# leggedrobotics/wild_visual_navigation

Hardware: AMD Instinct MI355X
Metric: frames/sec (448x448 DINO-ViT-S/8 + seg + MLP train-step) (higher is better)
Workload: dtype fp16 + e5m2-MX-correction linears (a w = a_h w_h + 2^-12 (a_h8 w_l8 + a_l8 w_h8); ~16 significand bits per product) + f16 attention products (two-plane q in the first six blocks), fp32 accumulate / residual (<= 1e-3 parity mode)

## Files before the change

wild_visual_navigation_amd/csrc/gemm_a384_x3.hip:

```cpp
#include <stdlib.h>

#include <algorithm>
#include <type_traits>

#include "common.h"
#include "wvn_internal.h"

namespace {

constexpr int KD = 384;
constexpr int BNT = 64;
constexpr int SLK = 128;
constexpr int NSL = KD / SLK;
constexpr int NS = 3;
constexpr int PLANE_BYTES = BNT * SLK * 2;
constexpr int SLICE_BYTES = 2 * PLANE_BYTES;
constexpr int RING_BYTES = NS * SLICE_BYTES;
constexpr int IMG_BF16 = 32 * 144;
constexpr int STG_BYTES = 2 * 64 * 80;
constexpr int STG_OFF = RING_BYTES;
constexpr int BIAS_OFF = STG_OFF + 4 * STG_BYTES;
constexpr int BM = 128;
constexpr int PIECES = SLICE_BYTES / 1024 / 4;
static_assert(PIECES == 8, "one DMA piece per k-step of a slice");
// ... 327 lines not shown
      if constexpr (TR) {
        const int c = 32 * t + 8 * g + 4 * hi + h2;
        if constexpr (EPI == X_GELU || EPI == X_GELU_FRAG) gelu_pair(v0, v1);
        if constexpr (EPI == X_GELU_FRAG && MX) {
          typedef __attribute__((ext_vector_type(2))) _Float16 h2_t;
          const uint32_t h = pack_f16x2(v0, v1);
          const h2_t hh = __builtin_bit_cast(h2_t, h);
          fragh[2 * (g & 1) + (h2 >> 1)] = h;
          {
            typedef __attribute__((ext_vector_type(2))) float f2_t;
            const f2_t res = f2_t{v0, v1} - f2_t{(float)hh[0], (float)hh[1]};
            frag8l[s >> 1] = mx_pk8(frag8l[s >> 1], res[0], res[1], MX_RES_INV, s & 1);
          }
          if ((s & 3) == 3) {
            const unsigned so = __builtin_amdgcn_readfirstlane((((m0w >> 5) * (p.N >> 4)) + 4 * jp + 2 * t + (g >> 1)) * 1024);
            wvn_store_b128_guarded(fragh, rs_c, lane * 16, so);
          }
          if (s == 7) {
            const unsigned so8 = __builtin_amdgcn_readfirstlane((((m0w >> 5) * (p.N >> 6)) + jp) * 2048 + t * 1024);
            wvn_store_b128_guarded(frag8l, rs_c2, lane * 16, so8);
          }
          return;
        }
        if constexpr (EPI == X_GELU_FRAG) {
          uint32_t h, l;
          split2(v0, v1, h, l);
          const int e = 2 * (g & 1) + (h2 >> 1);
          fragh[e] = h; fragl[e] = l;
          if ((s & 3) == 3) {
            const unsigned so = __builtin_amdgcn_readfirstlane((((m0w >> 5) * (p.N >> 4)) + 4 * jp + 2 * t + (g >> 1)) * 1024);
            wvn_store_b128_guarded(fragh, rs_c, lane * 16, so);
            wvn_store_b128_guarded(fragl, rs_c2, lane * 16, so);
          }
          return;
        }
        if constexpr (HEAD) {
          const wvn_f32x2_t b2 = *(const wvn_f32x2_t*)(bias_l + n0 + c);
          v0 += b2[0]; v1 += b2[1];
        }
        if constexpr (HEAD && !CODE) { v0 = fmaxf(v0, 0.f); v1 = fmaxf(v1, 0.f); }
        if constexpr (CODE) {
          const wvn_f32x2_t o = {v0, v1};
          *(wvn_f32x2_t*)(stg + l31 * 272 + c * 4) = o;
        } else if constexpr (EPI == X_RESID) {
          if (p.ls) { v0 *= p.ls[n0 + c]; v1 *= p.ls[n0 + c + 1]; }
          const wvn_f32x2_t o = {v0, v1};
          *(wvn_f32x2_t*)(stg + l31 * 272 + c * 4) = o;
        } else if constexpr (IS_QKV && F16OUT) {
          const float qs = n0 < p.heads * 64 ? p.q_scale : 1.f;
          uint32_t h, l;
          wvn_split2_f16(v0 * qs, v1 * qs, h, l);
          *(uint32_t*)(stg + l31 * 144 + c * 2) = h;
          *(uint32_t*)(stg + IMG_BF16 + l31 * 144 + c * 2) = l;
        } else {
          uint32_t h, l;
          split2(v0, v1, h, l);
          *(uint32_t*)(stg + l31 * 144 + c * 2) = h;
          *(uint32_t*)(stg + IMG_BF16 + l31 * 144 + c * 2) = l;
        }
      } else {
        const int mloc = 16 * (g >> 1) + 8 * hi + 4 * (g & 1) + h2;
        if constexpr (F16OUT) {
          *(uint32_t*)(stg + (32 * t + l31) * 80 + mloc * 2) = pack_f16x2(v0, v1);
        } else {
          uint32_t h, l;
          split2(v0, v1, h, l);
          *(uint32_t*)(stg + (32 * t + l31) * 80 + mloc * 2) = h;
          *(uint32_t*)(stg + 64 * 80 + (32 * t + l31) * 80 + mloc * 2) = l;
        }
      }
      return;
    }
    if constexpr (CODE) {
      const int it = s;
      const unsigned so = __builtin_amdgcn_readfirstlane(((m0w + 4 * it) * p.ld_code + (n0 - KD)) * 4);
      const u32x4_t o = *(const u32x4_t*)(stg + stg_rd_code + it * 4 * 272);
      const unsigned vo = m0w + 4 * it + (lane >> 4) < p.M ? voff[1] : OOB;
      wvn_store_b128_guarded(o, rs_code, vo, so);
    } else if constexpr (EPI == X_RESID) {
      const int it = s;
      const unsigned so = __builtin_amdgcn_readfirstlane(((m0w + 4 * it) * p.ldc + n0) * 4);
      f32x4_t v = *(const f32x4_t*)(stg + stg_rd + it * 4 * 272);
      const u32x4_t r = resid_q[it & 1];
      if (it + 2 < 8)
        resid_q[it & 1] = __builtin_amdgcn_raw_buffer_load_b128(rs_c, voff[0], __builtin_amdgcn_readfirstlane(((m0w + 4 * (it + 2)) * p.ldc + n0) * 4), 0);
#pragma unroll
      for (int e = 0; e < 4; ++e) v[e] += __uint_as_float(r[e]);
      u32x4_t o;
#pragma unroll
      for (int e = 0; e < 4; ++e) o[e] = __float_as_uint(v[e]);
      wvn_store_b128_guarded(o, rs_c, voff[0], so);
    } else if constexpr (IS_QKV && TR) {
      const int it = s & 3, pl = s >> 2;
      const int D = p.heads * 64;
      const int which = n0 / D, head = (n0 - which * D) >> 6;
      const unsigned so = __builtin_amdgcn_readfirstlane((which == 0 ? p.q_off : p.k_off) + head * p.npad * 64 * 2);
      const u32x4_t val = *(const u32x4_t*)(stg + pl * IMG_BF16 + ((lane >> 3) + it * 8) * 144 + (lane & 7) * 16);
      if (pl == 0) wvn_store_b128_guarded(val, rs_c, voff[it >> 1], so + (it & 1) * 1024);
      else {
        const bool keep = !F16OUT || (which == 0 && p.q_lo_f16);
        wvn_store_b128_guarded(val, rs_c2, keep ? voff[it >> 1] : OOB, so + (it & 1) * 1024);
      }
    } else if constexpr (IS_QKV && !TR) {
      const int it = s & 3, pl = s >> 2;
      if (pl == 1 && F16OUT) return;
      const int head = (MERGED ? n0 - 2 * p.heads * 64 : n0) >> 6;
      const u32x4_t val = *(const u32x4_t*)(stg + pl * 64 * 80 + ((lane >> 2) + it * 16) * 80 + (lane & 3) * 16);
      const unsigned so = __builtin_amdgcn_readfirstlane(p.v_off + (head * 64 + it * 16) * p.npad * 2);
      if (pl == 0) wvn_store_b128_guarded(val, rs_c, vt_off, so);
      else wvn_store_b128_guarded(val, rs_c2, vt_off, so);
    } else if constexpr (EPI == X_GELU_FRAG) {
    } else {
      const int it = s >> 1, pl = s & 1;
      const unsigned so = __builtin_amdgcn_readfirstlane(((m0w + 8 * it) * p.ldc + n0) * 2);
      const u32x4_t val = *(const u32x4_t*)(stg + pl * IMG_BF16 + stg_rd + it * 8 * 144);
      const unsigned vo = m0w + 8 * it + (lane >> 3) < p.M ? voff[0] : OOB;
      if (pl == 0) wvn_store_b128_guarded(val, rs_c, vo, so);
      else wvn_store_b128_guarded(val, rs_c2, vo, so);
    }
  };

  auto init_acc = [&](int j, auto tr_tag) __attribute__((always_inline)) {
    constexpr bool TR = decltype(tr_tag)::value;
    const int n0 = j * BNT;
    if constexpr (HEAD) {
#pragma unroll
      for (int t = 0; t < 2; ++t)
#pragma unroll
        for (int r = 0; r < 16; ++r) acc[t][r] = 0.f;
    } else if constexpr (TR) {
#pragma unroll
      for (int t = 0; t < 2; ++t)
#pragma unroll
        for (int g = 0; g < 4; ++g) {
          const f32x4_t b4 = *(const f32x4_t*)(bias_l + n0 + 32 * t + 8 * g + 4 * hi);
#pragma unroll
          for (int e = 0; e < 4; ++e) acc[t][4 * g + e] = b4[e];
        }
    } else {
#pragma unroll
      for (int t = 0; t < 2; ++t) {
        const float b = bias_l[n0 + 32 * t + l31];
#pragma unroll
        for (int r = 0; r < 16; ++r) acc[t][r] = b;
      }
    }
  };

  constexpr int ST2 = EPI == X_RESID ? 14 : (EPI == X_GELU || EPI == X_PLANES ? 8 : (EPI == X_GELU_FRAG ? 0 : (F16OUT ? 4 : 8)));
  constexpr int ST01 = EPI == X_GELU_FRAG ? (MX ? 3 : 4) : 0;
  long long t_wait = 0, t_iss = 0, t_mfma = 0;
  const long long t_start = TIMING ? (long long)__builtin_amdgcn_s_memtime() : 0;
  auto period = [&](int i, int ks, int j, bool stores_in_window, auto mtr, auto etr, auto epi_tag) __attribute__((always_inline)) {
    constexpr bool do_epi = decltype(epi_tag)::value;
    long long c0 = 0, c1 = 0, c2 = 0;
    if constexpr (TIMING) c0 = (long long)__builtin_amdgcn_s_memtime();
    if (i + 1 < total) {
      if (ks == 0 && stores_in_window && ST2 > 0) asm volatile("s_waitcnt vmcnt(%0)" ::"n"(PIECES + ST2) : "memory");
      else if (ks != 0 && do_epi && ST01 > 0) asm volatile("s_waitcnt vmcnt(%0)" ::"n"(PIECES + ST01) : "memory");
      else asm volatile("s_waitcnt vmcnt(%0)" ::"n"(PIECES) : "memory");
    } else {
      asm volatile("s_waitcnt vmcnt(0)" ::: "memory");
    }
    __builtin_amdgcn_s_barrier();
    if constexpr (TIMING) c1 = (long long)__builtin_amdgcn_s_memtime();
    issue_begin();
    __builtin_amdgcn_sched_barrier(0);
    if constexpr (TIMING) c2 = (long long)__builtin_amdgcn_s_memtime();
    if constexpr (BURST) {
#pragma unroll
      for (int s = 0; s < 8; ++s) issue_piece(i + NS - 1, s);
      __builtin_amdgcn_sched_barrier(0);
    }
    frag_read(i % NS, 0, 0);
#pragma unroll
    for (int s = 0; s < 8; ++s) {
      if constexpr (MX) {
        if (s + 1 < 8) frag_read(i % NS, s + 1, (s & 1) ^ 1);
        __builtin_amdgcn_sched_barrier(0);
      }
      if constexpr (!BURST) issue_piece(i + NS - 1, s);
      mfma_step(i % NS, ks, s, mtr);
      if constexpr (do_epi) epi_chunk(ks, j - 1, s, etr);
      if constexpr (MX) {
#pragma unroll
        for (int n = 0; n < 2; ++n) {
          __builtin_amdgcn_sched_group_barrier(0x008, 1, 0);
          __builtin_amdgcn_sched_group_barrier(0x002, 8, 0);
          __builtin_amdgcn_sched_group_barrier(0x200, 2, 0);
          __builtin_amdgcn_sched_group_barrier(0x030, 1, 0);
        }
        __builtin_amdgcn_sched_group_barrier(0x008, 1, 0);
        __builtin_amdgcn_sched_group_barrier(0x002, 24, 0);
        __builtin_amdgcn_sched_group_barrier(0x200, 2, 0);
        __builtin_amdgcn_sched_group_barrier(0x030, 2, 0);
      } else {
#pragma unroll
      for (int n = 0; n < 6; ++n) {
        __builtin_amdgcn_sched_group_barrier(0x008, 1, 0);
        __builtin_amdgcn_sched_group_barrier(0x100, 1, 0);
        __builtin_amdgcn_sched_group_barrier(0x002, 7, 0);
        __builtin_amdgcn_sched_group_barrier(0x200, 1, 0);
        __builtin_amdgcn_sched_group_barrier(0x030, 1, 0);
      }
      }
      __builtin_amdgcn_sched_barrier(0);
    }
    issue_end();
    if constexpr (TIMING) { t_wait += c1 - c0; t_iss += c2 - c1; t_mfma += (long long)__builtin_amdgcn_s_memtime() - c2; }
  };
  int si = 0;
  auto tile = [&](int j, int jj, int j_end, auto mtr, auto etr, auto next_tr) __attribute__((always_inline)) {
    if (jj >= 1) {
#pragma unroll
      for (int ks = 0; ks < NSL; ++ks) period(si + ks, ks, j, jj >= 2, mtr, etr, std::true_type{});
    } else {
#pragma unroll
      for (int ks = 0; ks < NSL; ++ks) period(si + ks, ks, j, false, mtr, etr, std::false_type{});
    }
    si += NSL;
#pragma unroll
    for (int t = 0; t < 2; ++t) prev[t] = acc[t];
    if (j + 1 < j_end) init_acc(j + 1, next_tr);
  };

  __syncthreads();
  for (int u = u_begin; u < u_end;) {
    const int rb = u / NT, j0 = u - rb * NT, j1 = min(NT, j0 + (u_end - u));
    m0w = rb * BM + wave * 32;
    if constexpr (TIMING) {
      const long long l0 = (long long)__builtin_amdgcn_s_memtime();
      load_a();
      asm volatile("s_waitcnt vmcnt(0)" ::: "memory");
      t_iss += (long long)__builtin_amdgcn_s_memtime() - l0;
    } else {
      load_a();
    }
    if constexpr (IS_QKV) qkv_offsets();
    if constexpr (MERGED) {
      using T = std::true_type; using F = std::false_type;
      if (j0 < nqk) init_acc(j0, T{}); else init_acc(j0, F{});
      for (int j = j0; j < j1; ++j) {
        if (j + 1 < nqk) tile(j, j - j0, j1, T{}, T{}, T{});
        else if (j < nqk) tile(j, j - j0, j1, T{}, T{}, F{});
        else if (j == nqk) tile(j, j - j0, j1, F{}, T{}, F{});
        else tile(j, j - j0, j1, F{}, F{}, F{});
      }
      if (j1 - 1 < nqk) {
#pragma unroll
        for (int part = 0; part < 3; ++part)
#pragma unroll
          for (int c = 0; c < 8; ++c) epi_chunk(part, j1 - 1, c, T{});
      } else {
#pragma unroll
        for (int part = 0; part < 3; ++part)
#pragma unroll
          for (int c = 0; c < 8; ++c) epi_chunk(part, j1 - 1, c, F{});
      }
    } else if constexpr (HEAD) {
      using T = std::true_type; using F = std::false_type;
      constexpr int NPL = KD / BNT;
      init_acc(j0, T{});
      for (int j = j0; j < j1; ++j) {
        if (j <= NPL) tile(j, j - j0, j1, T{}, T{}, T{});
        else tile(j, j - j0, j1, T{}, F{}, T{});
      }
      if (j1 - 1 < NPL) {
#pragma unroll
        for (int part = 0; part < 3; ++part)
#pragma unroll
          for (int c = 0; c < 8; ++c) epi_chunk(part, j1 - 1, c, T{});
      } else {
#pragma unroll
        for (int part = 0; part < 3; ++part)
#pragma unroll
          for (int c = 0; c < 8; ++c) epi_chunk(part, j1 - 1, c, F{});
      }
    } else {
      init_acc(j0, TRK{});
      for (int j = j0; j < j1; ++j) tile(j, j - j0, j1, TRK{}, TRK{}, TRK{});
#pragma unroll
      for (int part = 0; part < 3; ++part)
#pragma unroll
        for (int c = 0; c < 8; ++c) epi_chunk(part, j1 - 1, c, TRK{});
    }
    u += j1 - j0;
  }
  asm volatile("s_waitcnt vmcnt(0)" ::: "memory");
  if constexpr (TIMING) {
    if (lane == 0 && p.dbg) {
      long long* d = p.dbg + ((size_t)blockIdx.x * 4 + wave) * 4;
      d[0] = t_wait; d[1] = t_iss; d[2] = t_mfma; d[3] = (long long)__builtin_amdgcn_s_memtime() - t_start;
    }
  }
}


constexpr int S2_BN = 32;
constexpr int S2_NSL = 3;
constexpr int S2_NS = 3;
constexpr int S2_SLICE = 16384;
constexpr int S2_RING = S2_NS * S2_SLICE;
constexpr int S2_PIECES = S2_SLICE / 1024 / 4;
constexpr int S2_STG = 5120;
static_assert(S2_PIECES == 4, "one DMA piece per region");

template <int EPI, bool TIMING = false>
__global__ __launch_bounds__(256, 2) void gemm_a384_mx2_kernel(X384Params p) {
  static_assert(EPI == X_GELU_FRAG || EPI == X_QKV_F16, "fc1 + GELU -> MX planes, or q | k | v^T fp16");
  constexpr bool IS_QKV = EPI == X_QKV_F16;
  wvn_fp16_saturate();
  extern __shared__ __attribute__((aligned(16))) unsigned char smem[];
  const int tid = threadIdx.x, lane = tid & 63;
  const int wave = __builtin_amdgcn_readfirstlane(tid >> 6);
  const int l31 = lane & 31, hi = lane >> 5;
  const int NT = p.N / S2_BN;
  const int NRB = (p.M + BM - 1) / BM;
  const long long U = (long long)NRB * NT;
  const int u_begin = (int)(U * blockIdx.x / gridDim.x), u_end = (int)(U * (blockIdx.x + 1) / gridDim.x);
  const int total = (u_end - u_begin) * S2_NSL;
  constexpr int STG_OFF2 = S2_RING;
  constexpr int BIAS_OFF2 = STG_OFF2 + (IS_QKV ? 4 * S2_STG : 0);
  unsigned char* stg = smem + STG_OFF2 + wave * S2_STG;
  const float* bias_l = (const float*)(smem + BIAS_OFF2);
  const float* gam_l = (const float*)(smem + BIAS_OFF2 + p.N * 4);
  int m0w = 0;

  const __amdgpu_buffer_rsrc_t rs_w = __builtin_amdgcn_make_buffer_rsrc((void*)p.W, 0, (unsigned)((size_t)p.N * KD * 4), 0x00020000);
  const unsigned l16 = lane * 16;
  const int n_slices = NT * S2_NSL;
  int iss_g = (u_begin % NT) * S2_NSL;
  unsigned iss_soff = 0;
  auto issue_begin = [&]() __attribute__((always_inline)) { iss_soff = __builtin_amdgcn_readfirstlane((unsigned)iss_g * (unsigned)S2_SLICE + wave * S2_PIECES * 1024); };
  auto issue_piece = [&](int i, int u) __attribute__((always_inline)) {
    unsigned char* dst = smem + (i % S2_NS) * S2_SLICE + wave * S2_PIECES * 1024;
    __attribute__((address_space(3))) void* d3 = (__attribute__((address_space(3))) void*)dst;
    switch (u) {
      case 0: __builtin_amdgcn_raw_ptr_buffer_load_lds(rs_w, d3, 16, l16, iss_soff, 0, 0); break;
      case 1: __builtin_amdgcn_raw_ptr_buffer_load_lds(rs_w, d3, 16, l16, iss_soff, 1024, 0); break;
      case 2: __builtin_amdgcn_raw_ptr_buffer_load_lds(rs_w, d3, 16, l16, iss_soff, 2048, 0); break;
      default: __builtin_amdgcn_raw_ptr_buffer_load_lds(rs_w, d3, 16, l16, iss_soff, 3072, 0); break;
    }
  };
  auto issue_end = [&]() __attribute__((always_inline)) { if (++iss_g == n_slices) iss_g = 0; };
#pragma unroll
  for (int i = 0; i < S2_NS - 1; ++i)
    if (i < total) {
      issue_begin();
#pragma unroll
      for (int u = 0; u < S2_PIECES; ++u) issue_piece(i, u);
      issue_end();
    }
  for (int i = tid; i < p.N; i += 256) ((float*)(smem + BIAS_OFF2))[i] = p.bias ? p.bias[i] : 0.f;
  for (int i = tid; i < 2 * KD; i += 256) ((float*)(smem + BIAS_OFF2 + p.N * 4))[i] = i < KD ? p.ln_g[i] : p.ln_b[i - KD];

  u32x4_t mh[KD / 16];
  u32x4_t m8[KD / 64][2];
  auto load_a = [&]() __attribute__((always_inline)) {
    const int row = min(m0w + l31, p.M - 1);
    const wvn_f32x2_t st = *(const wvn_f32x2_t*)(p.ln_stats + 2 * (size_t)row);
    const float a1 = st[1], a0 = -st[0] * st[1];
    const float* xr = p.ln_x + (size_t)row * p.ln_ldx + hi * 8;
    constexpr int G = 8;
#pragma unroll
    for (int s0 = 0; s0 < KD / 16; s0 += G) {
      f32x4_t u[2 * G];
      __builtin_amdgcn_sched_barrier(0);
#pragma unroll
      for (int i = 0; i < G; ++i) {
        u[2 * i] = *(const f32x4_t*)(xr + (s0 + i) * 16);
        u[2 * i + 1] = *(const f32x4_t*)(xr + (s0 + i) * 16 + 4);
      }
      __builtin_amdgcn_sched_barrier(0);
#pragma unroll
      for (int i = 0; i < G; ++i) {
        const int s = s0 + i;
        const f32x4_t g0 = *(const f32x4_t*)(gam_l + s * 16 + hi * 8), g1 = *(const f32x4_t*)(gam_l + s * 16 + hi * 8 + 4);
        const f32x4_t b0 = *(const f32x4_t*)(gam_l + KD + s * 16 + hi * 8), b1 = *(const f32x4_t*)(gam_l + KD + s * 16 + hi * 8 + 4);
        float y[8];
#pragma unroll
        for (int e = 0; e < 4; ++e) {
          y[e] = fmaf(fmaf(u[2 * i][e], a1, a0), g0[e], b0[e]);
          y[4 + e] = fmaf(fmaf(u[2 * i + 1][e], a1, a0), g1[e], b1[e]);
        }
        u32x4_t hv;
        uint32_t d8[2] = {0, 0};
#pragma unroll
        for (int e = 0; e < 4; ++e) {
          typedef __attribute__((ext_vector_type(2))) _Float16 h2_t;
          const uint32_t hb = pack_f16x2(y[2 * e], y[2 * e + 1]);
          hv[e] = hb;
          const h2_t hh = __builtin_bit_cast(h2_t, hb);
          d8[e >> 1] = mx_pk8(d8[e >> 1], y[2 * e] - (float)hh[0], y[2 * e + 1] - (float)hh[1], MX_RES_INV, e & 1);
        }
        asm volatile("" : "+v"(hv), "+v"(d8[0]), "+v"(d8[1]));
        mh[s] = hv;
        m8[s >> 2][(s >> 1) & 1][2 * (s & 1)] = d8[0];
        m8[s >> 2][(s >> 1) & 1][2 * (s & 1) + 1] = d8[1];
        __builtin_amdgcn_sched_barrier(0);
      }
    }
  };

  f32x16_t acc;
#pragma unroll
  for (int r = 0; r < 16; ++r) acc[r] = 0.f;

  constexpr unsigned OOB = 0x80000000u;
  const int nqk = IS_QKV ? 4 * p.heads : (1 << 30);
  unsigned voff[2] = {0, 0};
  unsigned vt_off = 0;
  const unsigned c_bytes = IS_QKV ? 0u : (unsigned)((size_t)((p.M + 31) / 32 * 32) * p.ldc * 2);
  const __amdgpu_buffer_rsrc_t rs_c = IS_QKV ? __builtin_amdgcn_make_buffer_rsrc(p.qkv_base, 0, p.qkv_bytes, 0x00020000)
                                             : __builtin_amdgcn_make_buffer_rsrc(p.C, 0, c_bytes, 0x00020000);
  const __amdgpu_buffer_rsrc_t rs_c2 = IS_QKV ? __builtin_amdgcn_make_buffer_rsrc(p.qkv_base_lo ? p.qkv_base_lo : p.qkv_base, 0, p.qkv_bytes, 0x00020000)
                                              : __builtin_amdgcn_make_buffer_rsrc(p.C_lo ? p.C_lo : p.C, 0, c_bytes / 2, 0x00020000);
  auto qkv_offsets = [&]() __attribute__((always_inline)) {
#pragma unroll
    for (int hblk = 0; hblk < 2; ++hblk) {
      const int m = m0w + hblk * 16 + (lane >> 2);
      const int b = m / p.ntok_s, tk = m - b * p.ntok_s;
      voff[hblk] = m < p.M ? (unsigned)((((size_t)b * p.heads * p.npad + tk) * 64 + (lane & 3) * 8) * 2) : OOB;
    }
    {
      const int m = m0w + (lane & 3) * 8;
      const int b = m / p.ntok_s, tk = m - b * p.ntok_s;
      vt_off = m < p.M ? (unsigned)((((size_t)b * p.heads * 64 + (lane >> 2)) * p.npad + tk) * 2) : OOB;
    }
  };

  u32x4_t wq[2][2], w8[2][2];
  u32x4_t dh8[2] = {{0, 0, 0, 0}, {0, 0, 0, 0}};
  auto frag_read = [&](int slot, int r, int par) __attribute__((always_inline)) {
    const unsigned char* base = smem + slot * S2_SLICE + l16;
#pragma unroll
    for (int x = 0; x < 2; ++x) wq[par][x] = *(const u32x4_t*)(base + (2 * r + x) * 1024);
#pragma unroll
    for (int x = 0; x < 2; ++x) w8[par][x] = *(const u32x4_t*)(base + 8192 + (8 * (r >> 1) + 4 * (r & 1) + 2 * x) * 512);
  };
  auto derive_h8 = [&](int c) __attribute__((always_inline)) {
    typedef __attribute__((ext_vector_type(2))) _Float16 h2_t;
#pragma unroll
    for (int sfr = 0; sfr < 4; ++sfr) {
      uint32_t d[2] = {0, 0};
#pragma unroll
      for (int e = 0; e < 4; ++e) {
        const uint32_t pr = mh[c * 4 + sfr][e];
        const s16x2_t o = __builtin_bit_cast(s16x2_t, d[e >> 1]);
        d[e >> 1] = __builtin_bit_cast(uint32_t, (e & 1) ? __builtin_amdgcn_cvt_scalef32_pk_bf8_f16(o, __builtin_bit_cast(h2_t, pr), 1.0f, true)
                                                         : __builtin_amdgcn_cvt_scalef32_pk_bf8_f16(o, __builtin_bit_cast(h2_t, pr), 1.0f, false));
      }
      dh8[sfr >> 1][2 * (sfr & 1)] = d[0];
      dh8[sfr >> 1][2 * (sfr & 1) + 1] = d[1];
    }
  };
  auto mfma_region = [&](int ks, int r, int par, auto tr_tag) __attribute__((always_inline)) {
    constexpr bool TR = decltype(tr_tag)::value;
    const int c = 2 * ks + (r >> 1), which = r & 1;
#pragma unroll
    for (int x = 0; x < 2; ++x) {
      const f16x8_t af = __builtin_bit_cast(f16x8_t, mh[ks * 8 + 2 * r + x]);
      const f16x8_t wf = __builtin_bit_cast(f16x8_t, wq[par][x]);
      if constexpr (TR) acc = __builtin_amdgcn_mfma_f32_32x32x16_f16(wf, af, acc, 0, 0, 0);
      else acc = __builtin_amdgcn_mfma_f32_32x32x16_f16(af, wf, acc, 0, 0, 0);
    }
    const u32x4_t a0 = which ? m8[c][0] : dh8[0], a1 = which ? m8[c][1] : dh8[1];
    const i32x8_t av = {(int)a0[0], (int)a0[1], (int)a0[2], (int)a0[3], (int)a1[0], (int)a1[1], (int)a1[2], (int)a1[3]};
    const u32x4_t w0 = w8[par][0], w1 = w8[par][1];
    const i32x8_t wv = {(int)w0[0], (int)w0[1], (int)w0[2], (int)w0[3], (int)w1[0], (int)w1[1], (int)w1[2], (int)w1[3]};
    if constexpr (TR) acc = __builtin_amdgcn_mfma_scale_f32_32x32x64_f8f6f4(wv, av, acc, 1, 1, 0, which ? MX_SC_ONE : MX_SC_RES, 0, which ? MX_SC_RES : MX_SC_ONE);
    else acc = __builtin_amdgcn_mfma_scale_f32_32x32x64_f8f6f4(av, wv, acc, 1, 1, 0, which ? MX_SC_RES : MX_SC_ONE, 0, which ? MX_SC_ONE : MX_SC_RES);
  };

  auto init_acc = [&](int j, auto tr_tag) __attribute__((always_inline)) {
    constexpr bool TR = decltype(tr_tag)::value;
    const int n0 = j * S2_BN;
    if constexpr (TR) {
#pragma unroll
      for (int g = 0; g < 4; ++g) {
        const f32x4_t b4 = *(const f32x4_t*)(bias_l + n0 + 8 * g + 4 * hi);
#pragma unroll
        for (int e = 0; e < 4; ++e) acc[4 * g + e] = b4[e];
      }
    } else {
      const float b = bias_l[n0 + l31];
#pragma unroll
      for (int r = 0; r < 16; ++r) acc[r] = b;
    }
  };

  auto epilogue = [&](int j, auto tr_tag) __attribute__((always_inline)) {
    constexpr bool TR = decltype(tr_tag)::value;
    const int n0 = j * S2_BN;
    if constexpr (!IS_QKV) {
      const int jp = j >> 1, t = j & 1;
      u32x4_t frag8l = {0, 0, 0, 0};
#pragma unroll
      for (int gg = 0; gg < 2; ++gg) {
        u32x4_t fragh;
#pragma unroll
        for (int c = 0; c < 4; ++c) {
          const int s = 4 * gg + c, g = s >> 1, h2 = (s & 1) * 2;
          float v0 = acc[4 * g + h2], v1 = acc[4 * g + h2 + 1];
          gelu_pair(v0, v1);
          typedef __attribute__((ext_vector_type(2))) _Float16 h2_t;
          typedef __attribute__((ext_vector_type(2))) float f2_t;
          const uint32_t h = pack_f16x2(v0, v1);
          const h2_t hh = __builtin_bit_cast(h2_t, h);
          fragh[2 * (g & 1) + (h2 >> 1)] = h;
          const f2_t res = f2_t{v0, v1} - f2_t{(float)hh[0], (float)hh[1]};
          frag8l[s >> 1] = mx_pk8(frag8l[s >> 1], res[0], res[1], MX_RES_INV, s & 1);
        }
        const unsigned so = __builtin_amdgcn_readfirstlane((((m0w >> 5) * (p.N >> 4)) + 4 * jp + 2 * t + gg) * 1024);
        wvn_store_b128_guarded(fragh, rs_c, l16, so);
      }
      const unsigned so8 = __builtin_amdgcn_readfirstlane((((m0w >> 5) * (p.N >> 6)) + jp) * 2048 + t * 1024);
      wvn_store_b128_guarded(frag8l, rs_c2, l16, so8);
    } else if constexpr (TR) {
      const int D = p.heads * 64;
      const int which = n0 / D, head = (n0 - which * D) >> 6, t = (n0 >> 5) & 1;
      const float qs = which == 0 ? p.q_scale : 1.f;
      const bool keep_lo = which == 0 && p.q_lo_f16;
      const unsigned so = __builtin_amdgcn_readfirstlane((which == 0 ? p.q_off : p.k_off) + head * p.npad * 64 * 2 + t * 64);
#pragma unroll
      for (int g = 0; g < 4; ++g)
#pragma unroll
        for (int h2 = 0; h2 < 4; h2 += 2) {
          uint32_t h, l;
          wvn_split2_f16(acc[4 * g + h2] * qs, acc[4 * g + h2 + 1] * qs, h, l);
          const int c = 8 * g + 4 * hi + h2;
          *(uint32_t*)(stg + l31 * 80 + c * 2) = h;
          *(uint32_t*)(stg + 2560 + l31 * 80 + c * 2) = l;
          __builtin_amdgcn_sched_barrier(0);
        }
#pragma unroll
      for (int it = 0; it < 2; ++it) {
        const u32x4_t val = *(const u32x4_t*)(stg + ((lane >> 2) + it * 16) * 80 + (lane & 3) * 16);
        wvn_store_b128_guarded(val, rs_c, voff[it], so);
      }
      if (keep_lo) {
#pragma unroll
        for (int it = 0; it < 2; ++it) {
          const u32x4_t val = *(const u32x4_t*)(stg + 2560 + ((lane >> 2) + it * 16) * 80 + (lane & 3) * 16);
          wvn_store_b128_guarded(val, rs_c2, voff[it], so);
        }
      }
    } else {
      const int nv = n0 - 2 * p.heads * 64;
#pragma unroll
      for (int g = 0; g < 4; ++g)
#pragma unroll
        for (int h2 = 0; h2 < 4; h2 += 2) {
          const int mloc = 16 * (g >> 1) + 8 * hi + 4 * (g & 1) + h2;
          *(uint32_t*)(stg + l31 * 80 + mloc * 2) = pack_f16x2(acc[4 * g + h2], acc[4 * g + h2 + 1]);
        }
#pragma unroll
      for (int it = 0; it < 2; ++it) {
        const u32x4_t val = *(const u32x4_t*)(stg + ((lane >> 2) + it * 16) * 80 + (lane & 3) * 16);
        const unsigned so = __builtin_amdgcn_readfirstlane(p.v_off + (nv + it * 16) * p.npad * 2);
        wvn_store_b128_guarded(val, rs_c, vt_off, so);
      }
    }
  };

  long long t_bar = 0, t_loop = 0, t_epi = 0, t_pro = 0;
  const long long t_start = TIMING ? (long long)__builtin_amdgcn_s_memtime() : 0;
  auto period = [&](int i, int ks, auto tr_tag) __attribute__((always_inline)) {
    long long c0 = 0, c1 = 0, c2 = 0;
    if constexpr (TIMING) c0 = (long long)__builtin_amdgcn_s_memtime();
    __builtin_amdgcn_s_barrier();
    if constexpr (TIMING) c1 = (long long)__builtin_amdgcn_s_memtime();
    issue_begin();
    frag_read(i % S2_NS, 0, 0);
#pragma unroll
    for (int r = 0; r < 4; ++r) {
      if (r + 1 < 4) frag_read(i % S2_NS, r + 1, (r & 1) ^ 1);
      issue_piece(i + S2_NS - 1, r);
      if ((r & 1) == 0) derive_h8(2 * ks + (r >> 1));
      __builtin_amdgcn_sched_barrier(0);
      mfma_region(ks, r, r & 1, tr_tag);
      __builtin_amdgcn_sched_barrier(0);
    }
    issue_end();
    if constexpr (TIMING) c2 = (long long)__builtin_amdgcn_s_memtime();
    asm volatile("s_waitcnt vmcnt(%0)" ::"n"(S2_PIECES) : "memory");
    if constexpr (TIMING) { t_bar += c1 - c0 + (long long)__builtin_amdgcn_s_memtime() - c2; t_loop += c2 - c1; }
  };
  int si = 0;
  auto tile = [&](int j, bool last, auto tr_tag, auto next_tr) __attribute__((always_inline)) {
#pragma unroll
    for (int ks = 0; ks < S2_NSL; ++ks) period(si + ks, ks, tr_tag);
    si += S2_NSL;
    const long long e0 = TIMING ? (long long)__builtin_amdgcn_s_memtime() : 0;
    epilogue(j, tr_tag);
    if (!last) init_acc(j + 1, next_tr);
    if constexpr (TIMING) t_epi += (long long)__builtin_amdgcn_s_memtime() - e0;
  };

  __syncthreads();
  for (int u = u_begin; u < u_end;) {
    const int rb = u / NT, j0 = u - rb * NT, j1 = min(NT, j0 + (u_end - u));
    m0w = rb * BM + wave * 32;
    const long long l0 = TIMING ? (long long)__builtin_amdgcn_s_memtime() : 0;
    load_a();
    if constexpr (IS_QKV) qkv_offsets();
    asm volatile("s_waitcnt vmcnt(0)" ::: "memory");
    if constexpr (TIMING) t_pro += (long long)__builtin_amdgcn_s_memtime() - l0;
    using T = std::true_type; using F = std::false_type;
    if constexpr (IS_QKV) {
      if (j0 < nqk) {
        const int je = min(j1, nqk);
        init_acc(j0, T{});
        for (int j = j0; j < je; ++j) tile(j, j + 1 == je, T{}, T{});
      }
      if (j1 > nqk) {
        const int jb = max(j0, nqk);
        init_acc(jb, F{});
        for (int j = jb; j < j1; ++j) tile(j, j + 1 == j1, F{}, F{});
      }
    } else {
      init_acc(j0, T{});
      for (int j = j0; j < j1; ++j) tile(j, j + 1 == j1, T{}, T{});
    }
    u += j1 - j0;
  }
  asm volatile("s_waitcnt vmcnt(0)" ::: "memory");
  if constexpr (TIMING) {
    if (lane == 0 && p.dbg) {
      long long* d = p.dbg + ((size_t)blockIdx.x * 4 + wave) * 4;
      d[0] = t_bar; d[1] = t_pro; d[2] = t_loop; d[3] = (long long)__builtin_amdgcn_s_memtime() - t_start;
      (void)t_epi;
    }
  }
}

bool g_x384_split_qkv = getenv("WVN_X384_SPLIT_QKV") != nullptr;

int x384_num_cus() {
  static int n = 0;
  if (n == 0) {
    int dev = 0;
    hipDeviceProp_t prop;
    if (hipGetDevice(&dev) == hipSuccess && hipGetDeviceProperties(&prop, dev) == hipSuccess) n = prop.multiProcessorCount;
    if (n <= 0) n = 256;
  }
  return n;
}

template <int EPI>
int launch_mx(const X384Params& p, hipStream_t st) {
  if (!p.ln_x || !p.ln_stats || !p.ln_g || !p.ln_b || (p.ln_ldx % 4) || ((uintptr_t)p.ln_x & 15) || ((uintptr_t)p.ln_stats & 7)) return WVN_ERR_ARG;
  const int lds = BIAS_OFF + p.N * 4 + 2 * KD * 4;
  if (lds > X384_LDS_MAX) return WVN_ERR_ARG;
  static LdsOptIn lds_opt_in;
  if (const int rc = lds_opt_in(X384_LDS_MAX, (const void*)gemm_a384_x3_kernel<EPI, false, true, true>, (const void*)gemm_a384_x3_kernel<EPI, true, true, true>)) return rc;
  const long long units = (long long)ceil_div(p.M, BM) * (p.N / BNT);
  const int grid = (int)(units < x384_num_cus() ? units : x384_num_cus());
  static const bool burst = getenv("WVN_A384_MX_BURST") != nullptr;
  if (burst) {
    static LdsOptIn lds_opt_in_b;
    if (const int rc = lds_opt_in_b(X384_LDS_MAX, (const void*)gemm_a384_x3_kernel<EPI, false, true, true, true>, (const void*)gemm_a384_x3_kernel<EPI, true, true, true, true>)) return rc;
    if (p.dbg) hipLaunchKernelGGL((gemm_a384_x3_kernel<EPI, true, true, true, true>), dim3(grid), dim3(256), lds, st, p);
    else hipLaunchKernelGGL((gemm_a384_x3_kernel<EPI, false, true, true, true>), dim3(grid), dim3(256), lds, st, p);
    WVN_LAUNCH_CHECK();
    return WVN_OK;
  }
  if (p.dbg) hipLaunchKernelGGL((gemm_a384_x3_kernel<EPI, true, true, true>), dim3(grid), dim3(256), lds, st, p);
  else hipLaunchKernelGGL((gemm_a384_x3_kernel<EPI, false, true, true>), dim3(grid), dim3(256), lds, st, p);
  WVN_LAUNCH_CHECK();
  return WVN_OK;
}

template <int EPI>
int launch_mx2(X384Params p, hipStream_t st) {
  if (!p.ln_x || !p.ln_stats || !p.ln_g || !p.ln_b || (p.ln_ldx % 4) || ((uintptr_t)p.ln_x & 15) || ((uintptr_t)p.ln_stats & 7)) return WVN_ERR_ARG;
  p.W = (const bf16_t*)((const unsigned char*)p.W + (size_t)p.N * KD * 4);
  const int lds = S2_RING + (EPI == X_QKV_F16 ? 4 * S2_STG : 0) + p.N * 4 + 2 * KD * 4;
  if (lds > 80 * 1024) return WVN_ERR_ARG;
  static LdsOptIn lds_opt_in;
  if (const int rc = lds_opt_in(80 * 1024, (const void*)gemm_a384_mx2_kernel<EPI>, (const void*)gemm_a384_mx2_kernel<EPI, true>)) return rc;
  const long long units = (long long)ceil_div(p.M, BM) * (p.N / S2_BN);
  static const bool one_per_cu = getenv("WVN_A384_MX2_ONE") != nullptr;
  const int cap = (one_per_cu ? 1 : 2) * x384_num_cus();
  const int grid = (int)(units < cap ? units : cap);
  if (p.dbg) hipLaunchKernelGGL((gemm_a384_mx2_kernel<EPI, true>), dim3(grid), dim3(256), lds, st, p);
  else hipLaunchKernelGGL((gemm_a384_mx2_kernel<EPI>), dim3(grid), dim3(256), lds, st, p);
  WVN_LAUNCH_CHECK();
  return WVN_OK;
}

int g_a384_mx_form = [] { const char* e = getenv("WVN_A384_MX_FORM"); return e && e[0] == '2' ? 2 : (e && e[0] == '1' ? 1 : 0); }();

template <int EPI>
int launch(const X384Params& p, hipStream_t st) {
  constexpr bool CAN_LNA = EPI == X_QKV || EPI == X_QKV_F16 || EPI == X_GELU_FRAG;
  const bool lna = p.ln_x != nullptr;
  if (lna && (!CAN_LNA || !p.ln_stats || !p.ln_g || !p.ln_b || (p.ln_ldx % 4) || ((uintptr_t)p.ln_x & 15) || ((uintptr_t)p.ln_stats & 7))) return WVN_ERR_ARG;
  const int lds = BIAS_OFF + p.N * 4 + (lna ? 2 * KD * 4 : 0);
  if (lds > X384_LDS_MAX) return WVN_ERR_ARG;
  static LdsOptIn lds_opt_in;
  if (const int rc = lds_opt_in(X384_LDS_MAX, (const void*)gemm_a384_x3_kernel<EPI>, (const void*)gemm_a384_x3_kernel<EPI, true>)) return rc;
  const long long units = (long long)ceil_div(p.M, BM) * (p.N / BNT);
  const int grid = (int)(units < x384_num_cus() ? units : x384_num_cus());
  if constexpr (CAN_LNA) {
    if (lna) {
      static LdsOptIn lds_opt_in_lna;
      if (const int rc = lds_opt_in_lna(X384_LDS_MAX, (const void*)gemm_a384_x3_kernel<EPI, false, true>)) return rc;
      hipLaunchKernelGGL((gemm_a384_x3_kernel<EPI, false, true>), dim3(grid), dim3(256), lds, st, p);
      WVN_LAUNCH_CHECK();
      return WVN_OK;
    }
  }
  if (p.dbg) hipLaunchKernelGGL((gemm_a384_x3_kernel<EPI, true>), dim3(grid), dim3(256), lds, st, p);
  else hipLaunchKernelGGL((gemm_a384_x3_kernel<EPI>), dim3(grid), dim3(256), lds, st, p);
  WVN_LAUNCH_CHECK();
  return WVN_OK;
}

}

int wvn_gemm_a384_x3_launch(const GemmBf16Params& g, int epi, hipStream_t st) {
  const bool lna = g.ln_x != nullptr;
  if (g.K != KD || g.ldw != KD || (g.N % BNT) != 0 || g.M <= 0 || !g.W || !g.W_lo) return WVN_ERR_ARG;
  if (!lna && (!g.A || !g.A_lo || (g.lda % 8) != 0 || (((uintptr_t)g.A | (uintptr_t)g.A_lo) & 15))) return WVN_ERR_ARG;
  if (((uintptr_t)g.W | (uintptr_t)g.W_lo) & 15) return WVN_ERR_ARG;
  if (g.W_lo <= g.W || (size_t)(g.W_lo - g.W) + (size_t)g.N * KD >= (1ull << 30)) return WVN_ERR_ARG;
  X384Params p{};
  p.A = g.A; p.A_lo = g.A_lo; p.lda = g.lda; p.W = g.W; p.w_plane = (size_t)(g.W_lo - g.W); p.bias = g.bias;
  p.C = g.C; p.C_lo = g.C_lo; p.ldc = g.ldc; p.M = g.M; p.N = g.N;
  p.heads = g.heads; p.npad = g.npad; p.ntok_s = g.ntok_s; p.q_scale = g.q_scale != 0.f ? g.q_scale : 1.f; p.f16_out = g.qkv_f16;
  p.ls = g.ls; p.dbg = g.dbg;
  p.ln_x = g.ln_x; p.ln_ldx = g.ln_ldx; p.ln_stats = g.ln_stats; p.ln_g = g.ln_g; p.ln_b = g.ln_b;
  switch (epi) {
    case EPI_GELU_BF16:
      if (!g.C || !g.C_lo || (g.ldc % 8) != 0 || (((uintptr_t)g.C | (uintptr_t)g.C_lo) & 15) || (size_t)g.M * g.ldc * 2 >= (1ull << 31)) return WVN_ERR_ARG;
      return launch<X_GELU>(p, st);
    case EPI_GELU_FRAG:
      if (!g.C || !g.C_lo || g.ldc != g.N || (((uintptr_t)g.C | (uintptr_t)g.C_lo) & 15) || ((size_t)g.M + 32) * g.ldc * 2 >= (1ull << 31)) return WVN_ERR_ARG;
      return launch<X_GELU_FRAG>(p, st);
    case EPI_BF16:
      if (!g.C || !g.C_lo || (g.ldc % 8) != 0 || (((uintptr_t)g.C | (uintptr_t)g.C_lo) & 15) || (size_t)g.M * g.ldc * 2 >= (1ull << 31)) return WVN_ERR_ARG;
      return launch<X_PLANES>(p, st);
    case EPI_RESID_F32:
    case EPI_ACCUM_F32:
      if (!g.C || (g.ldc % 4) != 0 || ((uintptr_t)g.C & 15) || (size_t)g.M * g.ldc * 4 >= (1ull << 31)) return WVN_ERR_ARG;
      return launch<X_RESID>(p, st);
    case EPI_QKV: {
      if (g.N != 3 * g.heads * 64 || !g.q || !g.k || !g.vt || (g.ntok_s % 16) || (g.M % 16) || (g.npad % 16)) return WVN_ERR_ARG;
      if (!g.qkv_f16 && (!g.q_lo || !g.k_lo || !g.vt_lo)) return WVN_ERR_ARG;
      const uintptr_t lo = std::min({(uintptr_t)g.q, (uintptr_t)g.k, (uintptr_t)g.vt});
      const uintptr_t hi = std::max({(uintptr_t)g.q, (uintptr_t)g.k, (uintptr_t)g.vt});
      const size_t one = (size_t)(g.M / (g.ntok_s > 0 ? g.ntok_s : 1)) * g.heads * g.npad * 64 * 2;
      if (hi - lo + one >= (1ull << 31)) return WVN_ERR_ARG;
      p.qkv_base = (bf16_t*)lo; p.q_off = (unsigned)((uintptr_t)g.q - lo); p.k_off = (unsigned)((uintptr_t)g.k - lo);
      p.v_off = (unsigned)((uintptr_t)g.vt - lo); p.qkv_bytes = (unsigned)(hi - lo + one);
      if (g.qkv_f16 && g.q_lo) {
        if ((uintptr_t)g.q_lo < p.q_off) return WVN_ERR_ARG;
        p.qkv_base_lo = (bf16_t*)((uintptr_t)g.q_lo - p.q_off);
        p.q_lo_f16 = 1;
      }
      if (!g.qkv_f16) {
        const uintptr_t lo2 = std::min({(uintptr_t)g.q_lo, (uintptr_t)g.k_lo, (uintptr_t)g.vt_lo});
        if ((uintptr_t)g.q_lo - lo2 != p.q_off || (uintptr_t)g.k_lo - lo2 != p.k_off || (uintptr_t)g.vt_lo - lo2 != p.v_off) return WVN_ERR_ARG;
        p.qkv_base_lo = (bf16_t*)lo2;
      }
      const int D = g.heads * 64;
      if (!g_x384_split_qkv || lna) return g.qkv_f16 ? launch<X_QKV_F16>(p, st) : launch<X_QKV>(p, st);
      p.N = 2 * D;
      const int rc = g.qkv_f16 ? launch<X_QK_F16>(p, st) : launch<X_QK>(p, st);
      if (rc != WVN_OK) return rc;
      p.W = g.W + (size_t)2 * D * KD;
      p.bias = g.bias ? g.bias + 2 * D : nullptr;
      p.N = D;
      return g.qkv_f16 ? launch<X_V_F16>(p, st) : launch<X_V>(p, st);
    }
    default: return WVN_ERR_ARG;
  }
}

int wvn_gemm_a384_head_launch(const float* x, int ldx, const float* stats, const float* g, const float* b, const bf16_t* W, const bf16_t* W_lo, const float* bias,
                              bf16_t* hid, bf16_t* hid_lo, float* code, int ld_code, int frames, int npatch, int ntok_s, hipStream_t st) {
  constexpr int N = KD + 2 * BNT;
  if (!x || !stats || !g || !b || !W || !W_lo || !bias || !hid || !hid_lo || !code) return WVN_ERR_ARG;
  if (frames <= 0 || npatch <= 0 || ntok_s <= npatch || (ldx % 4) || ldx < KD || (ld_code % 4) || ld_code < 2 * BNT) return WVN_ERR_ARG;
  if (((uintptr_t)x | (uintptr_t)W | (uintptr_t)W_lo | (uintptr_t)hid | (uintptr_t)hid_lo | (uintptr_t)code) & 15) return WVN_ERR_ARG;
  if ((uintptr_t)stats & 7) return WVN_ERR_ARG;
  if (W_lo <= W || (size_t)(W_lo - W) + (size_t)N * KD >= (1ull << 30)) return WVN_ERR_ARG;
  const long long M = (long long)frames * npatch;
  if (M * KD * 2 >= (1ll << 31) || M * ld_code * 4 >= (1ll << 31)) return WVN_ERR_ARG;
  X384Params p{};
  p.lda = KD; p.W = W; p.w_plane = (size_t)(W_lo - W); p.bias = bias;
  p.C = hid; p.C_lo = hid_lo; p.ldc = KD; p.M = (int)M; p.N = N; p.q_scale = 1.f;
  p.ntok_s = ntok_s; p.npatch = npatch; p.code = code; p.ld_code = ld_code;
  p.ln_x = x; p.ln_ldx = ldx; p.ln_stats = stats; p.ln_g = g; p.ln_b = b;
  const int lds = BIAS_OFF + N * 4 + 2 * KD * 4;
  static_assert(BIAS_OFF + N * 4 + 2 * KD * 4 <= X384_LDS_MAX, "ring + staging + bias / gamma / beta tables");
  static LdsOptIn lds_opt_in;
  if (const int rc = lds_opt_in(X384_LDS_MAX, (const void*)gemm_a384_x3_kernel<X_HEAD, false, true>)) return rc;
  const long long units = (long long)ceil_div(p.M, BM) * (N / BNT);
  const int grid = (int)(units < x384_num_cus() ? units : x384_num_cus());
  hipLaunchKernelGGL((gemm_a384_x3_kernel<X_HEAD, false, true>), dim3(grid), dim3(256), lds, st, p);
  WVN_LAUNCH_CHECK();
  return WVN_OK;
}

void wvn_gemm_a384_mx_set_form(int form) { g_a384_mx_form = form == 1 || form == 2 ? form : 0; }

int wvn_gemm_a384_mx_launch(const GemmBf16Params& g, int epi, hipStream_t st) {
  if (!g.ln_x || g.K != KD || g.ldw != KD || (g.N % BNT) != 0 || g.M <= 0 || !g.W || !g.W_lo) return WVN_ERR_ARG;
  if (((uintptr_t)g.W | (uintptr_t)g.W_lo) & 15) return WVN_ERR_ARG;
  if (g.W_lo <= g.W || (size_t)(g.W_lo - g.W) + (size_t)g.N * KD >= (1ull << 30)) return WVN_ERR_ARG;
  X384Params p{};
  p.lda = KD; p.W = g.W; p.w_plane = (size_t)(g.W_lo - g.W); p.bias = g.bias;
  p.C = g.C; p.C_lo = g.C_lo; p.C_h8 = g.C_h8; p.ldc = g.ldc; p.M = g.M; p.N = g.N;
  p.heads = g.heads; p.npad = g.npad; p.ntok_s = g.ntok_s; p.q_scale = g.q_scale != 0.f ? g.q_scale : 1.f; p.f16_out = 1;
  p.dbg = g.dbg;
  p.ln_x = g.ln_x; p.ln_ldx = g.ln_ldx; p.ln_stats = g.ln_stats; p.ln_g = g.ln_g; p.ln_b = g.ln_b;
  switch (epi) {
    case EPI_GELU_FRAG:
      if (!g.C || !g.C_lo || g.ldc != g.N || (g.N % 64) || (((uintptr_t)g.C | (uintptr_t)g.C_lo) & 15) || ((size_t)g.M + 32) * g.ldc * 2 >= (1ull << 31))
        return WVN_ERR_ARG;
      return g_a384_mx_form != 1 ? launch_mx2<X_GELU_FRAG>(p, st) : launch_mx<X_GELU_FRAG>(p, st);
    case EPI_QKV: {
      if (!g.qkv_f16 || g.N != 3 * g.heads * 64 || !g.q || !g.k || !g.vt || (g.ntok_s % 16) || (g.M % 16) || (g.npad % 16)) return WVN_ERR_ARG;
      const uintptr_t lo = std::min({(uintptr_t)g.q, (uintptr_t)g.k, (uintptr_t)g.vt});
      const uintptr_t hi = std::max({(uintptr_t)g.q, (uintptr_t)g.k, (uintptr_t)g.vt});
      const size_t one = (size_t)(g.M / (g.ntok_s > 0 ? g.ntok_s : 1)) * g.heads * g.npad * 64 * 2;
      if (hi - lo + one >= (1ull << 31)) return WVN_ERR_ARG;
      p.qkv_base = (bf16_t*)lo; p.q_off = (unsigned)((uintptr_t)g.q - lo); p.k_off = (unsigned)((uintptr_t)g.k - lo);
      p.v_off = (unsigned)((uintptr_t)g.vt - lo); p.qkv_bytes = (unsigned)(hi - lo + one);
      if (g.q_lo) {
        if ((uintptr_t)g.q_lo < p.q_off) return WVN_ERR_ARG;
        p.qkv_base_lo = (bf16_t*)((uintptr_t)g.q_lo - p.q_off);
        p.q_lo_f16 = 1;
      }
      return g_a384_mx_form != 1 ? launch_mx2<X_QKV_F16>(p, st) : launch_mx<X_QKV_F16>(p, st);
    }
    default: return WVN_ERR_ARG;
  }
}
```

Baseline: 896.5.

## Store QKV epilogue directly from registers via permlane32 swaps, drop LDS staging

The QKV fp16 epilogue of the mx2 GEMM no longer transposes accumulator fragments through a per-wave LDS staging buffer. q/k tiles are written straight from registers using permlane32_swap to form 16-byte rows, and v^T tiles are stored directly with per-lane transposed offsets. Token-to-batch offset math is restructured to use wave-uniform bases. This removes LDS writes, reads and the staging region (20KB), which may also relax LDS pressure, but it changes the store access pattern and the bounds handling.

```diff
diff --git a/wild_visual_navigation_amd/csrc/gemm_a384_x3.hip b/wild_visual_navigation_amd/csrc/gemm_a384_x3.hip
--- a/wild_visual_navigation_amd/csrc/gemm_a384_x3.hip
+++ b/wild_visual_navigation_amd/csrc/gemm_a384_x3.hip
@@ -653,7 +653,6 @@
 constexpr int S2_SLICE = 16384;
 constexpr int S2_RING = S2_NS * S2_SLICE;
 constexpr int S2_PIECES = S2_SLICE / 1024 / 4;
-constexpr int S2_STG = 5120;
 static_assert(S2_PIECES == 4, "one DMA piece per region");
 
 template <int EPI, bool TIMING = false>
@@ -670,9 +669,7 @@
   const long long U = (long long)NRB * NT;
   const int u_begin = (int)(U * blockIdx.x / gridDim.x), u_end = (int)(U * (blockIdx.x + 1) / gridDim.x);
   const int total = (u_end - u_begin) * S2_NSL;
-  constexpr int STG_OFF2 = S2_RING;
-  constexpr int BIAS_OFF2 = STG_OFF2 + (IS_QKV ? 4 * S2_STG : 0);
-  unsigned char* stg = smem + STG_OFF2 + wave * S2_STG;
+  constexpr int BIAS_OFF2 = S2_RING;
   const float* bias_l = (const float*)(smem + BIAS_OFF2);
   const float* gam_l = (const float*)(smem + BIAS_OFF2 + p.N * 4);
   int m0w = 0;
@@ -759,24 +756,30 @@
 
   constexpr unsigned OOB = 0x80000000u;
   const int nqk = IS_QKV ? 4 * p.heads : (1 << 30);
-  unsigned voff[2] = {0, 0};
-  unsigned vt_off = 0;
+  unsigned qk_off = 0;
+  const unsigned vt_lane = IS_QKV ? (unsigned)(l31 * p.npad + 8 * hi) * 2u : 0u;
+  unsigned vt_so[2] = {0, 0};
+  bool vt_in[2] = {false, false};
   const unsigned c_bytes = IS_QKV ? 0u : (unsigned)((size_t)((p.M + 31) / 32 * 32) * p.ldc * 2);
   const __amdgpu_buffer_rsrc_t rs_c = IS_QKV ? __builtin_amdgcn_make_buffer_rsrc(p.qkv_base, 0, p.qkv_bytes, 0x00020000)
                                              : __builtin_amdgcn_make_buffer_rsrc(p.C, 0, c_bytes, 0x00020000);
   const __amdgpu_buffer_rsrc_t rs_c2 = IS_QKV ? __builtin_amdgcn_make_buffer_rsrc(p.qkv_base_lo ? p.qkv_base_lo : p.qkv_base, 0, p.qkv_bytes, 0x00020000)
                                               : __builtin_amdgcn_make_buffer_rsrc(p.C_lo ? p.C_lo : p.C, 0, c_bytes / 2, 0x00020000);
   auto qkv_offsets = [&]() __attribute__((always_inline)) {
-#pragma unroll
-    for (int hblk = 0; hblk < 2; ++hblk) {
-      const int m = m0w + hblk * 16 + (lane >> 2);
-      const int b = m / p.ntok_s, tk = m - b * p.ntok_s;
-      voff[hblk] = m < p.M ? (unsigned)((((size_t)b * p.heads * p.npad + tk) * 64 + (lane & 3) * 8) * 2) : OOB;
-    }
+    const int b0 = __builtin_amdgcn_readfirstlane(m0w / p.ntok_s), r0 = m0w - b0 * p.ntok_s;
     {
-      const int m = m0w + (lane & 3) * 8;
-      const int b = m / p.ntok_s, tk = m - b * p.ntok_s;
-      vt_off = m < p.M ? (unsigned)((((size_t)b * p.heads * 64 + (lane >> 2)) * p.npad + tk) * 2) : OOB;
+      int b = b0, tk = r0 + l31;
+#pragma unroll
+      for (int i = 0; i < 2; ++i)
+        if (tk >= p.ntok_s) { tk -= p.ntok_s; ++b; }
+      qk_off = m0w + l31 < p.M ? ((unsigned)(b * p.heads * p.npad + tk) * 128u + hi * 16) : OOB;
+    }
+#pragma unroll
+    for (int gg = 0; gg < 2; ++gg) {
+      const bool wrap = r0 + 16 * gg >= p.ntok_s;
+      const int b = b0 + wrap, tk = r0 + 16 * gg - (wrap ? p.ntok_s : 0);
+      vt_so[gg] = __builtin_amdgcn_readfirstlane((unsigned)(b * p.heads * 64 * p.npad + tk) * 2u);
+      vt_in[gg] = m0w + 16 * gg < p.M;
     }
   };
 
@@ -870,46 +873,47 @@
     } else if constexpr (TR) {
       const int D = p.heads * 64;
       const int which = n0 / D, head = (n0 - which * D) >> 6, t = (n0 >> 5) & 1;
-      const float qs = which == 0 ? p.q_scale : 1.f;
-      const bool keep_lo = which == 0 && p.q_lo_f16;
       const unsigned so = __builtin_amdgcn_readfirstlane((which == 0 ? p.q_off : p.k_off) + head * p.npad * 64 * 2 + t * 64);
-#pragma unroll
-      for (int g = 0; g < 4; ++g)
-#pragma unroll
-        for (int h2 = 0; h2 < 4; h2 += 2) {
-          uint32_t h, l;
-          wvn_split2_f16(acc[4 * g + h2] * qs, acc[4 * g + h2 + 1] * qs, h, l);
-          const int c = 8 * g + 4 * hi + h2;
-          *(uint32_t*)(stg + l31 * 80 + c * 2) = h;
-          *(uint32_t*)(stg + 2560 + l31 * 80 + c * 2) = l;
-          __builtin_amdgcn_sched_barrier(0);
-        }
-#pragma unroll
-      for (int it = 0; it < 2; ++it) {
-        const u32x4_t val = *(const u32x4_t*)(stg + ((lane >> 2) + it * 16) * 80 + (lane & 3) * 16);
-        wvn_store_b128_guarded(val, rs_c, voff[it], so);
-      }
-      if (keep_lo) {
-#pragma unroll
-        for (int it = 0; it < 2; ++it) {
-          const u32x4_t val = *(const u32x4_t*)(stg + 2560 + ((lane >> 2) + it * 16) * 80 + (lane & 3) * 16);
-          wvn_store_b128_guarded(val, rs_c2, voff[it], so);
-        }
-      }
+      auto put = [&](uint32_t (&w)[8], auto lo_tag) __attribute__((always_inline)) {
+#pragma unroll
+        for (int pr = 0; pr < 2; ++pr) {
+          const auto r0 = __builtin_amdgcn_permlane32_swap(w[4 * pr], w[4 * pr + 2], false, false);
+          const auto r1 = __builtin_amdgcn_permlane32_swap(w[4 * pr + 1], w[4 * pr + 3], false, false);
+          const u32x4_t val = {r0[0], r1[0], r0[1], r1[1]};
+          if constexpr (decltype(lo_tag)::value) wvn_store_b128_guarded(val, rs_c2, qk_off, so + pr * 32);
+          else wvn_store_b128_guarded(val, rs_c, qk_off, so + pr * 32);
+        }
+      };
+      auto body = [&](auto scale_tag, auto lo_tag, float qs) __attribute__((always_inline)) {
+        constexpr bool SCALE = decltype(scale_tag)::value, LO = decltype(lo_tag)::value;
+        typedef __attribute__((ext_vector_type(2))) _Float16 h2_t;
+        uint32_t h[8];
+        [[maybe_unused]] uint32_t l[8];
+#pragma unroll
+        for (int w = 0; w < 8; ++w) {
+          const float a = acc[2 * w], b = acc[2 * w + 1];
+          h[w] = SCALE ? pack_f16x2(a * qs, b * qs) : pack_f16x2(a, b);
+          if constexpr (LO) {
+            const h2_t hh = __builtin_bit_cast(h2_t, h[w]);
+            l[w] = pack_f16x2(__builtin_fmaf(a, qs, -(float)hh[0]), __builtin_fmaf(b, qs, -(float)hh[1]));
+          }
+        }
+        put(h, std::false_type{});
+        if constexpr (LO) put(l, std::true_type{});
+      };
+      using T = std::true_type; using F = std::false_type;
+      if (which != 0) body(F{}, F{}, 1.f);
+      else if (p.q_lo_f16) body(T{}, T{}, p.q_scale);
+      else body(T{}, F{}, p.q_scale);
     } else {
       const int nv = n0 - 2 * p.heads * 64;
-#pragma unroll
-      for (int g = 0; g < 4; ++g)
-#pragma unroll
-        for (int h2 = 0; h2 < 4; h2 += 2) {
-          const int mloc = 16 * (g >> 1) + 8 * hi + 4 * (g & 1) + h2;
-          *(uint32_t*)(stg + l31 * 80 + mloc * 2) = pack_f16x2(acc[4 * g + h2], acc[4 * g + h2 + 1]);
-        }
-#pragma unroll
-      for (int it = 0; it < 2; ++it) {
-        const u32x4_t val = *(const u32x4_t*)(stg + ((lane >> 2) + it * 16) * 80 + (lane & 3) * 16);
-        const unsigned so = __builtin_amdgcn_readfirstlane(p.v_off + (nv + it * 16) * p.npad * 2);
-        wvn_store_b128_guarded(val, rs_c, vt_off, so);
+      const unsigned so = __builtin_amdgcn_readfirstlane(p.v_off + nv * p.npad * 2);
+#pragma unroll
+      for (int gg = 0; gg < 2; ++gg) {
+        u32x4_t val;
+#pragma unroll
+        for (int c = 0; c < 4; ++c) val[c] = pack_f16x2(acc[8 * gg + 2 * c], acc[8 * gg + 2 * c + 1]);
+        if (vt_in[gg]) wvn_store_b128_guarded(val, rs_c, vt_lane, so + vt_so[gg]);
       }
     }
   };
@@ -1026,7 +1030,7 @@
 int launch_mx2(X384Params p, hipStream_t st) {
   if (!p.ln_x || !p.ln_stats || !p.ln_g || !p.ln_b || (p.ln_ldx % 4) || ((uintptr_t)p.ln_x & 15) || ((uintptr_t)p.ln_stats & 7)) return WVN_ERR_ARG;
   p.W = (const bf16_t*)((const unsigned char*)p.W + (size_t)p.N * KD * 4);
-  const int lds = S2_RING + (EPI == X_QKV_F16 ? 4 * S2_STG : 0) + p.N * 4 + 2 * KD * 4;
+  const int lds = S2_RING + p.N * 4 + 2 * KD * 4;
   if (lds > 80 * 1024) return WVN_ERR_ARG;
   static LdsOptIn lds_opt_in;
   if (const int rc = lds_opt_in(80 * 1024, (const void*)gemm_a384_mx2_kernel<EPI>, (const void*)gemm_a384_mx2_kernel<EPI, true>)) return rc;
```

After: 910.7 (median of 6 runs). +1.6%, better.
